# Sahar-E/NeRF-and-DietNeRF

Measured on AMD Instinct MI355X. Metric: rays/sec (coarse+fine) at 256x256, 64 coarse + 128 fine samples, higher is better.
Workload: dtype f16 (3-pass hi/lo split operands, f32 accumulate; fp32-class results)

## Files before the change

### nerf_and_dietnerf_amd/csrc/mlp_f16_frag.h

```cpp
#pragma once
#include "mlp_common.h"

namespace nerf {

typedef _Float16 h8 __attribute__((ext_vector_type(8)));
typedef _Float16 h2 __attribute__((ext_vector_type(2)));
typedef uint32_t frag4 __attribute__((ext_vector_type(4)));

template <int OFF>
__device__ __forceinline__ void lds_read_frag_asm(f32x4& dst, uint32_t base) {
    asm volatile("ds_read_b128 %0, %1 offset:%2" : "=a"(dst) : "v"(base), "n"(OFF) : "memory");
}
template <int N>
__device__ __forceinline__ void lds_wait_frag_asm(f32x4& reg) {
#ifdef NERF_DIAG_NO_LDSWAIT
    asm volatile("" : "+a"(reg) : : "memory");
#else
    asm volatile("s_waitcnt lgkmcnt(%1)" : "+a"(reg) : "n"(N) : "memory");
#endif
}

__device__ __forceinline__ uint32_t pack_h2(float a, float b) {
    const h2 t = {(_Float16)a, (_Float16)b};
    return __builtin_bit_cast(uint32_t, t);
}

constexpr int kHCQ = 32;
constexpr int kHRing = 4;
constexpr int kHChunkBytes = kHCQ * kQuadBytes;
static_assert(kHRing * kHChunkBytes == kRingBytes, "fp16 ring must fill the shared LDS carve");

__device__ __forceinline__ void split_trunc(float y, float& hi_f, float& lo_f) {
    hi_f = __uint_as_float(__float_as_uint(y) & 0xFFFFE000u);
    lo_f = y - hi_f;
}


#ifndef NERF_PE_LX
#define NERF_PE_LX 5
#endif
constexpr int kPeLx = NERF_PE_LX;
constexpr int kPeDim = 3 + 6 * kPeLx;
constexpr int kHStepsPE = (kPeDim + 15) / 16;
constexpr int kHStepsHid = 16;
constexpr int kHStepsDir = 2;
constexpr int kHQpuPE = 2 * kHStepsPE;
constexpr int kHQpuHid = 2 * kHStepsHid;
constexpr int kHQpuSkip = kHQpuPE + kHQpuHid;
constexpr int kHQpuLast = kHQpuHid + 2 * kHStepsDir;
constexpr int kHTilesLast = 5;
constexpr int kHChunksPE = (8 * kHQpuPE + kHCQ - 1) / kHCQ;
constexpr int kHChunksHid = (8 * kHQpuHid) / kHCQ;
constexpr int kHChunksSkip = (8 * kHQpuSkip + kHCQ - 1) / kHCQ;
constexpr int kHChunksLast = (kHTilesLast * kHQpuLast + kHCQ - 1) / kHCQ;
constexpr int kHStreamChunks = kHChunksPE + 6 * kHChunksHid + kHChunksSkip + kHChunksLast;
constexpr int kHChunksSig = (kHQpuLast + kHCQ - 1) / kHCQ;
constexpr int kHStreamChunksSig = kHStreamChunks - kHChunksLast + kHChunksSig;
static_assert(kHStreamChunksSig * (size_t)kHChunkBytes == kStreamBytesF16Sig, "sigma-only stream size mismatch");
constexpr int kFChunksPE = (8 * kHStepsPE + kHCQ - 1) / kHCQ;
constexpr int kFChunksHid = (8 * kHStepsHid) / kHCQ;
constexpr int kFChunksSkip = (8 * (kHStepsPE + kHStepsHid) + kHCQ - 1) / kHCQ;
constexpr int kFChunksLast = (kHTilesLast * (kHStepsHid + kHStepsDir) + kHCQ - 1) / kHCQ;
constexpr int kFStreamChunks = kFChunksPE + 6 * kFChunksHid + kFChunksSkip + kFChunksLast;
static_assert(kFStreamChunks * (size_t)kHChunkBytes == kStreamBytesF16Hi, "hi-only stream size mismatch");
constexpr int kHConstBias = 0;
constexpr int kHConstBias8 = 2048;
constexpr int kHConstBiasSig = 2176;
constexpr int kHConstWrgb = 2208;
constexpr int kHConstBHead = 2592;
constexpr int kHConstFloats = 2608;

static_assert(kHStreamChunks * (size_t)kHChunkBytes == kStreamBytesF16, "stream size mismatch");
constexpr int kXChunksHidSig = (9 * kHQpuHid) / kHCQ;
constexpr int kXChunksLast0 = (4 * kHQpuHid) / kHCQ;
constexpr int kXStreamChunks = kHChunksPE + 6 * kHChunksHid + kHChunksSkip + kXChunksHidSig + kXChunksLast0;
constexpr int kXFChunksHidSig = (9 * kHStepsHid + kHCQ - 1) / kHCQ;
constexpr int kXFChunksLast0 = (4 * kHStepsHid) / kHCQ;
constexpr int kXFStreamChunks = kFChunksPE + 6 * kFChunksHid + kFChunksSkip + kXFChunksHidSig + kXFChunksLast0;
static_assert(kXStreamChunks * (size_t)kHChunkBytes == kStreamBytesF16Xyz, "xyz-only stream size mismatch");
static_assert(kXFStreamChunks * (size_t)kHChunkBytes == kStreamBytesF16HiXyz, "xyz-only hi stream size mismatch");
constexpr int kXConstBiasSig = 2048;
constexpr int kXConstBias8 = 2080;
constexpr int kXConstBias9 = 2336;
constexpr int kXConstWrgb = 2464;
constexpr int kXConstBHead = 2848;
constexpr int kXConstWsig = 2864;
constexpr int kXConstFloats = 3120;
static_assert(kXConstFloats <= kConstFloats, "xyz-only constants must fit the shared LDS carve");
enum { BODY_HIDSIG = 4, BODY_LAST0 = 5, BODY_SIG = 6 };
static_assert(kHConstFloats <= kConstFloats, "f16x3 constants must fit the shared LDS carve");

template <class T>
__device__ __forceinline__ void stream_store(T* p, const T& v) {
#ifndef NERF_STASH_NO_NT
    __builtin_nontemporal_store(v, p);
#else
    *p = v;
#endif
}
__device__ __forceinline__ void stream_store(uint2* p, const uint2& v) {
    typedef uint32_t u32x2 __attribute__((ext_vector_type(2)));
    u32x2 w;
    w[0] = v.x; w[1] = v.y;
    stream_store(reinterpret_cast<u32x2*>(p), w);
}

__device__ __forceinline__ uint32_t mask_push(uint32_t word, uint32_t packed_pair) {
    return (packed_pair & 0x80008000u) | (word >> 1);
}
__host__ __device__ constexpr int mask_bit(int ut, int r) { return 8 * (ut & 1) + (r >> 1) + 16 * (r & 1); }

__host__ __device__ inline int frag_feature(int n, int e, int h) {
    const int t = n >> 1, s = n & 1;
    return 32 * t + 16 * s + 8 * (e >> 2) + 4 * h + (e & 3);
}

}
```

### nerf_and_dietnerf_amd/csrc/mlp_f16x3.hip

```cpp
#include "mlp_f16_frag.h"

#include <math.h>
#include <string.h>

#if defined(NERF_BF16) && NERF_PE_LX == 5
namespace nerf::bf16 {
#elif defined(NERF_BF16)
namespace nerf::bf16::wide {
#elif NERF_PE_LX == 5
namespace nerf {
#else
namespace nerf::wide {
#endif

#ifdef NERF_BF16
typedef __bf16 e8 __attribute__((ext_vector_type(8)));
typedef __bf16 bf2 __attribute__((ext_vector_type(2)));
#define NERF_MFMA_E16 __builtin_amdgcn_mfma_f32_32x32x16_bf16
__device__ __forceinline__ void split_e(float y, float& hi_f, float& lo_f) {
    hi_f = __uint_as_float(__float_as_uint(y) & 0xFFFF0000u);
    lo_f = y - hi_f;
}
__device__ __forceinline__ uint32_t pack_hi(float a, float b) {
    return __builtin_amdgcn_perm(__float_as_uint(b), __float_as_uint(a), 0x07060302u);
}
__device__ __forceinline__ uint32_t pack_lo(float a, float b) {
    const bf2 t = {(__bf16)a, (__bf16)b};
    return __builtin_bit_cast(uint32_t, t);
}
#else
typedef h8 e8;
#define NERF_MFMA_E16 __builtin_amdgcn_mfma_f32_32x32x16_f16
__device__ __forceinline__ void split_e(float y, float& hi_f, float& lo_f) { split_trunc(y, hi_f, lo_f); }
__device__ __forceinline__ uint32_t pack_hi(float a, float b) { return pack_h2(a, b); }
__device__ __forceinline__ uint32_t pack_lo(float a, float b) { return pack_h2(a, b); }
#endif

#ifdef NERF_STAMPS
__device__ unsigned long long g_stamps_h[16];
#endif

template <int BODY, bool PENDING, bool FAST, bool STASH = false, int ROT = 0>
__device__ __forceinline__ void layer_body_h(Pipe& p, uint32_t lane16, uint32_t cb_h, int bias_off_bytes,
                                             float alpha, float* st_prev, float* st_cur, frag4* mk_prev_ptr,
                                             frag4* mk_cur_ptr, frag4& mk_prev, frag4& mk_cur, f32x16 (&accs)[4],
                                             frag4 (&xh)[16], frag4 (&xl)[16], frag4 (&nh)[14], frag4 (&nl)[14],
                                             const frag4 (&peh)[kHStepsPE], const frag4 (&pel)[kHStepsPE], const frag4 (&dh)[2],
                                             const frag4 (&dl)[2], float (&xc)[64], float& sigma_raw) {
    constexpr int NU = BODY == BODY_LAST ? kHTilesLast : BODY == BODY_SIG ? 1 : BODY == BODY_HIDSIG ? 9 : BODY == BODY_LAST0 ? 4 : 8;
    constexpr int NSTEP = BODY == BODY_PE ? kHStepsPE : (BODY == BODY_HID || BODY == BODY_HIDSIG || BODY == BODY_LAST0) ? kHStepsHid
                          : BODY == BODY_SKIP ? kHStepsPE + kHStepsHid : kHStepsHid + kHStepsDir;
    constexpr int SIG0 = BODY == BODY_HIDSIG ? 1 : 0;
    constexpr int TPS = FAST ? 1 : 2;
    constexpr int QPU = TPS * NSTEP;
    constexpr int NQ = NU * QPU;
#ifndef NERF_KPF
#define NERF_KPF 4
#endif
#ifndef NERF_KPF_FAST
#define NERF_KPF_FAST 8
#endif
    constexpr int kPf = FAST ? NERF_KPF_FAST : NERF_KPF;
#ifndef NERF_STASH_EXTRA_FAST
#define NERF_STASH_EXTRA_FAST 0
#endif
#ifndef NERF_STASH_EXTRA_3P
#define NERF_STASH_EXTRA_3P 0
#endif
    constexpr int kStashExtra = STASH ? (FAST ? NERF_STASH_EXTRA_FAST : NERF_STASH_EXTRA_3P) : 0;
    f32x4 pf[kPf];
    const int ck0 = p.ck;
    uint32_t rdbase[2];
    rdbase[0] = lane16 + (uint32_t)((ck0 + 0) & (kHRing - 1)) * kHChunkBytes;
    rdbase[1] = lane16 + (uint32_t)((ck0 + 1) & (kHRing - 1)) * kHChunkBytes;
    auto issue_read = [&](auto qc) {
        constexpr int Qa = decltype(qc)::value;
        lds_read_frag_asm<(Qa % kHCQ) * kQuadBytes>(pf[Qa % kPf], rdbase[(Qa / kHCQ) & 1]);
    };
    static_for<0, kPf>([&](auto ic) {
        if constexpr (decltype(ic)::value < NQ) issue_read(ic);
    });

    auto act = [&](float v) -> float {
        const float av = alpha * v;
        float y;
        asm("v_max_f32 %0, %1, %2" : "=v"(y) : "v"(v), "v"(av));
        return y;
    };
    auto load_bias = [&](int off_bytes, f32x16& dst) {
        static_for<0, 4>([&](auto gc) {
            constexpr int g = decltype(gc)::value;
            const f32x4 b = lds_read4(cb_h + off_bytes + g * 32);
            dst[4 * g + 0] = b[0]; dst[4 * g + 1] = b[1]; dst[4 * g + 2] = b[2]; dst[4 * g + 3] = b[3];
        });
    };
    float sq0 = 0.f, sq1 = 0.f;
    (void)sq0; (void)sq1;
    auto stash4 = [&](auto utc, auto rc, float y0, float y1, float* base) {
        constexpr int ut = decltype(utc)::value;
        constexpr int r = decltype(rc)::value;
        if constexpr ((r & 3) == 0) { sq0 = y0; sq1 = y1; }
        else {
            f32x4 v;
            v[0] = sq0; v[1] = sq1; v[2] = y0; v[3] = y1;
#ifndef NERF_DIAG_NO_STASH_STORES
            stream_store(reinterpret_cast<f32x4*>(base + 32 * (32 * ut + 8 * (r >> 2))), v);
#else
            asm volatile("" :: "v"(v), "v"(base));
#endif
        }
    };
    uint32_t sqh = 0u;
    (void)sqh;
    auto stash4h = [&](auto utc, auto rc, uint32_t ph, float* base) {
        constexpr int ut = decltype(utc)::value;
        constexpr int r = decltype(rc)::value;
        if constexpr ((r & 3) == 0) sqh = ph;
#ifndef NERF_DIAG_NO_STASH_STORES
        else stream_store(reinterpret_cast<uint2*>(reinterpret_cast<uint16_t*>(base) + 32 * (32 * ut + 8 * (r >> 2))), make_uint2(sqh, ph));
#else
        else asm volatile("" :: "v"(sqh), "v"(ph), "v"(base));
#endif
    };
    auto store_pair = [&](auto utc, auto rc, float y0, float y1, auto dest_sel, auto pend_sel) {
        constexpr int ut = decltype(utc)::value;
        constexpr int r = decltype(rc)::value;
        constexpr int n = 2 * ut + (r >> 3), e = r & 7;
        uint32_t ph, pl = 0u;
        if constexpr (FAST) {
            ph = pack_h2(y0, y1);
        } else {
            float h0, l0, h1, l1;
            split_e(y0, h0, l0);
            split_e(y1, h1, l1);
            ph = pack_hi(h0, h1); pl = pack_lo(l0, l1);
        }
        if constexpr (STASH) {
            if constexpr (FAST) stash4h(utc, rc, ph, decltype(pend_sel)::value ? st_prev : st_cur);
            else stash4(utc, rc, y0, y1, decltype(pend_sel)::value ? st_prev : st_cur);
            if constexpr (decltype(pend_sel)::value) mk_prev[ut >> 1] = mask_push(mk_prev[ut >> 1], ph);
            else mk_cur[ut >> 1] = mask_push(mk_cur[ut >> 1], ph);
        }
        if constexpr (decltype(dest_sel)::value) { xh[n][e >> 1] = ph; if constexpr (!FAST) xl[n][e >> 1] = pl; }
        else { nh[n][e >> 1] = ph; if constexpr (!FAST) nl[n][e >> 1] = pl; }
    };

#ifndef NERF_FAST_PACKED_EPI
#define NERF_FAST_PACKED_EPI 1
#endif
    constexpr bool kPackedEpi = FAST && NERF_FAST_PACKED_EPI != 0;
    const uint32_t alpha2 = pack_h2(alpha, alpha);
    (void)alpha2;
    auto act_pair = [&](float v0, float v1) -> uint32_t {
        const uint32_t pk = pack_h2(v0, v1);
        uint32_t q, y;
        asm("v_pk_mul_f16 %0, %1, %2" : "=v"(q) : "v"(pk), "v"(alpha2));
        asm("v_pk_max_f16 %0, %1, %2" : "=v"(y) : "v"(pk), "v"(q));
        return y;
    };
    auto store_pair_p = [&](auto utc, auto rc, uint32_t ph, auto dest_sel, auto pend_sel) {
        constexpr int ut = decltype(utc)::value;
        constexpr int r = decltype(rc)::value;
        constexpr int n = 2 * ut + (r >> 3), e = r & 7;
        if constexpr (STASH) {
            stash4h(utc, rc, ph, decltype(pend_sel)::value ? st_prev : st_cur);
            if constexpr (decltype(pend_sel)::value) mk_prev[ut >> 1] = mask_push(mk_prev[ut >> 1], ph);
            else mk_cur[ut >> 1] = mask_push(mk_cur[ut >> 1], ph);
        }
        if constexpr (decltype(dest_sel)::value) xh[n][e >> 1] = ph;
        else nh[n][e >> 1] = ph;
    };
    (void)act_pair; (void)store_pair_p;
    float ycarry = 0.f;
    (void)ycarry;
    static_for<0, NU>([&](auto uc) {
        constexpr int u = decltype(uc)::value;
        f32x16& acc = accs[(u + ROT) & 3];
        f32x16& prv = accs[(u + ROT + 3) & 3];
        f32x16& nxt = accs[(u + ROT + 1) & 3];
        if constexpr (u == 0 && !PENDING) load_bias(bias_off_bytes, acc);
        static_for<0, NSTEP>([&](auto nc) {
            constexpr int n = decltype(nc)::value;
            f32x4 araw[2];
            static_for<0, TPS>([&](auto tc) {
                constexpr int t = decltype(tc)::value;
                constexpr int Q = u * QPU + TPS * n + t;
                constexpr int left = NQ - Q;
                (void)left;
                constexpr int qc = Q % kHCQ;
                if constexpr (qc == 0 && Q > 0) p.ck += 1;
                if constexpr (qc == kHCQ / 2) {
                    constexpr int room = (NQ - 1 - Q) / 2;
                    pipe_sync_c<kHCQ, kHRing, (room + 1 < kHCQ / 4 ? room + 1 : kHCQ / 4), kStashExtra>(p);
                }
                if constexpr (qc > kHCQ / 2 && (qc - kHCQ / 2) % 2 == 0) {
                    constexpr int Qs = Q - (qc - kHCQ / 2);
                    constexpr bool tail = (NQ - 1 - Qs) / 2 + 1 < kHCQ / 4;
                    pipe_piece_c<(qc - kHCQ / 2) / 2, tail>(p);
                }
                lds_wait_frag_asm<(NQ - Q >= kPf ? kPf - 1 : NQ - Q - 1)>(pf[Q % kPf]);
                araw[t] = pf[Q % kPf];
                if constexpr (Q + kPf < NQ) {
                    constexpr int Qn = Q + kPf;
                    if constexpr (Qn % kHCQ == 0)
                        rdbase[(Qn / kHCQ) & 1] = lane16 + (uint32_t)((ck0 + Qn / kHCQ) & (kHRing - 1)) * kHChunkBytes;
                    issue_read(std::integral_constant<int, Qn>{});
                }
            });
            const e8 a_hi = __builtin_bit_cast(e8, araw[0]);
            const e8 a_lo = __builtin_bit_cast(e8, araw[FAST ? 0 : 1]);
            (void)a_lo;
            frag4 bh_, bl_;
            if constexpr (BODY == BODY_PE) { bh_ = peh[n]; bl_ = pel[n]; }
            else if constexpr (BODY == BODY_HID || BODY == BODY_HIDSIG || BODY == BODY_LAST0) { bh_ = xh[n]; bl_ = xl[n]; }
            else if constexpr (BODY == BODY_SKIP) {
                if constexpr (n < kHStepsPE) { bh_ = peh[n]; bl_ = pel[n]; }
                else { bh_ = xh[n - kHStepsPE]; bl_ = xl[n - kHStepsPE]; }
            } else {
                if constexpr (n < kHStepsHid) { bh_ = xh[n]; bl_ = xl[n]; }
                else { bh_ = dh[n - kHStepsHid]; bl_ = dl[n - kHStepsHid]; }
            }
            const e8 b_hi = __builtin_bit_cast(e8, bh_), b_lo = __builtin_bit_cast(e8, bl_);
            constexpr bool kPend = (u == 0) && PENDING && n < 8;
            constexpr bool kPrevS = (u > SIG0) && BODY != BODY_PE && NSTEP >= 16 && n < 16;
            constexpr int et = kPend ? 7 : (u > SIG0 ? u - 1 - SIG0 : 0);
            constexpr bool kXc = (BODY == BODY_LAST || BODY == BODY_LAST0) && kPrevS;
            if constexpr (BODY == BODY_HIDSIG && u == 1 && n == 0) sigma_raw = prv[0];
            if constexpr (!FAST) {
                acc = NERF_MFMA_E16(a_hi, b_lo, acc, 0, 0, 0);
                acc = NERF_MFMA_E16(a_lo, b_hi, acc, 0, 0, 0);
            }
            acc = NERF_MFMA_E16(a_hi, b_hi, acc, 0, 0, 0);
            if constexpr (kPend && kPackedEpi) {
                constexpr int er = 2 * n;
                store_pair_p(std::integral_constant<int, 7>{}, std::integral_constant<int, er>{}, act_pair(prv[er], prv[er + 1]), std::true_type{}, std::true_type{});
            } else if constexpr (kPrevS && !kXc && kPackedEpi) {
                if constexpr ((n & 1) == 1)
                    store_pair_p(std::integral_constant<int, et>{}, std::integral_constant<int, n - 1>{}, act_pair(prv[n - 1], prv[n]), std::false_type{}, std::false_type{});
            } else if constexpr (kPend) {
                constexpr int er = 2 * n;
                const float y0 = act(prv[er]), y1 = act(prv[er + 1]);
                store_pair(std::integral_constant<int, 7>{}, std::integral_constant<int, er>{}, y0, y1, std::true_type{}, std::true_type{});
            } else if constexpr (kPrevS) {
                const float y = act(prv[n]);
                if constexpr (kXc) {
                    xc[et * 16 + n] = y;
                    if constexpr (STASH) {
                        if constexpr ((n & 1) == 0) ycarry = y;
                        else {
                            const uint32_t pp = pack_h2(ycarry, y);
                            if constexpr (FAST) stash4h(std::integral_constant<int, et>{}, std::integral_constant<int, n - 1>{}, pp, st_cur);
                            else stash4(std::integral_constant<int, et>{}, std::integral_constant<int, n - 1>{}, ycarry, y, st_cur);
                            mk_cur[et >> 1] = mask_push(mk_cur[et >> 1], pp);
                        }
                    }
                }
                else if constexpr ((n & 1) == 0) ycarry = y;
                else store_pair(std::integral_constant<int, et>{}, std::integral_constant<int, n - 1>{}, ycarry, y, std::false_type{}, std::false_type{});
            }
            if constexpr (u == 0 && PENDING) {
                if constexpr (STASH && n == 8) { if (mk_prev_ptr) stream_store(mk_prev_ptr, mk_prev); }
                if constexpr (n == 8) { xh[12] = nh[12]; xl[12] = nl[12]; }
                if constexpr (n == 9) { xh[13] = nh[13]; xl[13] = nl[13]; }
            }
            if constexpr (n == (NSTEP >= 12 ? 10 : 0)) {
                if constexpr (u + 1 < NU) load_bias(bias_off_bytes + (u + 1) * 128, nxt);
                else if constexpr (BODY != BODY_LAST && BODY != BODY_LAST0 && BODY != BODY_SIG) load_bias(bias_off_bytes + NU * 128, nxt);
            }
            if constexpr (BODY == BODY_PE && u > 0 && n == 0) {
                static_for<0, 8>([&](auto pc) {
                    constexpr int r = 2 * decltype(pc)::value;
                    if constexpr (kPackedEpi) {
                        const uint32_t ph = act_pair(prv[r], prv[r + 1]);
                        if constexpr (u - 1 <= 5) store_pair_p(std::integral_constant<int, u - 1>{}, std::integral_constant<int, r>{}, ph, std::true_type{}, std::false_type{});
                        else store_pair_p(std::integral_constant<int, u - 1>{}, std::integral_constant<int, r>{}, ph, std::false_type{}, std::false_type{});
                        return;
                    }
                    const float z0 = act(prv[r]), z1 = act(prv[r + 1]);
                    if constexpr (u - 1 <= 5) store_pair(std::integral_constant<int, u - 1>{}, std::integral_constant<int, r>{}, z0, z1, std::true_type{}, std::false_type{});
                    else store_pair(std::integral_constant<int, u - 1>{}, std::integral_constant<int, r>{}, z0, z1, std::false_type{}, std::false_type{});
                });
            }
            if constexpr ((BODY == BODY_HID || BODY == BODY_SKIP || BODY == BODY_HIDSIG) && u == NU - 1) {
                constexpr int m = BODY == BODY_SKIP ? n - kHStepsPE : n;
                if constexpr (m >= 1 && m - 1 < 12) { xh[m - 1] = nh[m - 1]; xl[m - 1] = nl[m - 1]; }
            }
        });
    });
    if constexpr (BODY == BODY_LAST0) {
        f32x16& lastacc = accs[(NU - 1 + ROT) & 3];
#pragma unroll
        for (int r = 0; r < 16; ++r) xc[(NU - 1) * 16 + r] = act(lastacc[r]);
        if constexpr (STASH) {
            static_for<0, 8>([&](auto pc) {
                constexpr int r = 2 * decltype(pc)::value;
                const float y0 = xc[(NU - 1) * 16 + r], y1 = xc[(NU - 1) * 16 + r + 1];
                const uint32_t pp = pack_h2(y0, y1);
                if constexpr (FAST) stash4h(std::integral_constant<int, NU - 1>{}, std::integral_constant<int, r>{}, pp, st_cur);
                else stash4(std::integral_constant<int, NU - 1>{}, std::integral_constant<int, r>{}, y0, y1, st_cur);
                mk_cur[(NU - 1) >> 1] = mask_push(mk_cur[(NU - 1) >> 1], pp);
            });
            if (mk_cur_ptr) stream_store(mk_cur_ptr, mk_cur);
        }
    }
    if constexpr (BODY == BODY_LAST || BODY == BODY_SIG) {
        static_assert(((NU - 1 + ROT) & 3) == 0, "the sigma tile's accumulator");
        sigma_raw = accs[(NU - 1) & 3][0];
        if constexpr (STASH) { if (mk_cur_ptr) stream_store(mk_cur_ptr, mk_cur); }
    }
    if constexpr (NQ % kHCQ != 0 && NQ % kHCQ <= kHCQ / 2) pipe_sync_c<kHCQ, kHRing, 1, kStashExtra>(p);
    p.ck += 1;
}

template <bool FAST>
__device__ __forceinline__ void split8(const float (&v)[8], frag4& hi, frag4& lo) {
#pragma unroll
    for (int e = 0; e < 8; e += 2) {
        if constexpr (FAST) {
            hi[e >> 1] = pack_h2(v[e], v[e + 1]);
            lo[e >> 1] = 0u;
            continue;
        }
        float h0, l0, h1, l1;
        split_e(v[e], h0, l0);
        split_e(v[e + 1], h1, l1);
        hi[e >> 1] = pack_hi(h0, h1);
        lo[e >> 1] = pack_lo(l0, l1);
    }
}

template <bool FAST, bool STASH = false, bool XYZ = false, bool SIGONLY = false>
__device__ __forceinline__ void mlp_f16_body(const MlpArgs& a) {
    static_assert(!SIGONLY || (!FAST && !STASH && !XYZ), "the sigma-only variant is a render kernel of the 3-pass network");
    extern __shared__ __attribute__((aligned(16))) char smem[];
    const int tid = threadIdx.x;
    const int lane = tid & 63;
    const int wave = __builtin_amdgcn_readfirstlane(tid >> 6);
    const int j = lane & 31;
    const int h = lane >> 5;
    const uint32_t lane16 = kLdsRing + lane * 16;
    uint32_t cb_h = kLdsConst + h * 16;
    asm volatile("" : "+v"(cb_h));

    const long long ntiles = (a.M + 127) / 128;
    if ((long long)blockIdx.x >= ntiles) return;

    for (int i = tid; i < (XYZ ? kXConstFloats : kHConstFloats) / 4; i += 256) {
        const bool sig = SIGONLY && i >= kHConstBias8 / 4 && i < (kHConstBias8 + 32) / 4;
        reinterpret_cast<f32x4*>(smem + kLdsConst)[i] =
            reinterpret_cast<const f32x4*>(a.wconst)[sig ? i + (kHConstBiasSig - kHConstBias8) / 4 : i];
    }

    Pipe p;
    p.ck = 0;
    p.src_next = 0;
    p.n_chunks = XYZ ? (FAST ? kXFStreamChunks : kXStreamChunks) : SIGONLY ? kHStreamChunksSig : (FAST ? kFStreamChunks : kHStreamChunks);
    p.wbase = reinterpret_cast<const char*>(a.wstream);
    p.voff = wave * (kHCQ / 4 * kQuadBytes) + lane * 16;
    p.wave_lds = wave * (kHCQ / 4 * kQuadBytes);
    __syncthreads();
#pragma unroll
    for (int c = 0; c < kHRing - 1; ++c) {
        p.cur_src = p.wbase + (size_t)p.src_next * kHChunkBytes;
        p.cur_dst = kLdsRing + c * kHChunkBytes + p.wave_lds;
        p.src_next += 1;
#pragma unroll
        for (int j = 0; j < kHCQ / 4; ++j) dma_piece(p.cur_src, p.voff + j * kQuadBytes, p.cur_dst + j * kQuadBytes);
    }
    asm volatile("s_waitcnt vmcnt(%0)" ::"n"((kHCQ / 4) * (kHRing - 2)) : "memory");
    __builtin_amdgcn_s_barrier();
    asm volatile("" ::: "memory");

    frag4 xh[16], xl[16], nh[14], nl[14], peh[kHStepsPE], pel[kHStepsPE], dh[2], dl[2];
    f32x16 accs[4];
    float xc[64];
    float sigma_raw = 0.f;

    unsigned long long t0 = 0, t1 = 0, acc_t[8] = {0, 0, 0, 0, 0, 0, 0, 0};
    (void)t0; (void)t1; (void)acc_t;
    for (long long tile = blockIdx.x; tile < ntiles; tile += gridDim.x) {
        STAMP(t0);
        const long long m = tile * 128 + wave * 32 + j;
        const bool valid = m < a.M;
        const long long mm = valid ? m : a.M - 1;
        float px, py, pz, dx, dy, dz;
        if (a.mode == 0) {
            const long long ray = mm / a.S;
            const f32x4 o = *reinterpret_cast<const f32x4*>(a.in_a + ray * 4);
            const f32x4 d = *reinterpret_cast<const f32x4*>(a.in_b + ray * 4);
            const float zz = a.z[mm];
            px = __fadd_rn(o[0], __fmul_rn(d[0], zz));
            py = __fadd_rn(o[1], __fmul_rn(d[1], zz));
            pz = __fadd_rn(o[2], __fmul_rn(d[2], zz));
            dx = d[0]; dy = d[1]; dz = d[2];
        } else {
            px = a.in_a[mm * 3 + 0]; py = a.in_a[mm * 3 + 1]; pz = a.in_a[mm * 3 + 2];
            if constexpr (XYZ) { dx = dy = dz = 0.f; }
            else { dx = a.in_b[mm * 3 + 0]; dy = a.in_b[mm * 3 + 1]; dz = a.in_b[mm * 3 + 2]; }
        }
        const float kPi = 3.1415927410125732f;
        float pv[8 * kHStepsPE];
#pragma unroll
        for (int c = 0; c < 3; ++c) {
            const float v = c == 0 ? px : c == 1 ? py : pz;
            if constexpr (FAST) {
                sin_ladder_fp16_modes<kPeLx>(v * kPi, h, &pv[c * kPeLx]);
            } else {
#pragma unroll
                for (int k = 0; k < kPeLx; ++k) pv[c * kPeLx + k] = sin_shifted(v * (kPi * (float)(1 << k)), h);
            }
        }
        if constexpr (kPeLx == 5) {
            pv[15] = h ? 0.f : px; pv[16] = h ? 0.f : py; pv[17] = h ? 0.f : pz;
#pragma unroll
            for (int i = 18; i < 24; ++i) pv[i] = 0.f;
        } else {
            static_assert(kPeLx == 10, "the wide-PE layout holds exactly 10 octaves");
            pv[30] = h ? pz : px; pv[31] = h ? 0.f : py;
        }
#pragma unroll
        for (int n = 0; n < kHStepsPE; ++n) {
            float t8[8];
#pragma unroll
            for (int e = 0; e < 8; ++e) t8[e] = pv[n * 8 + e];
            split8<FAST>(t8, peh[n], pel[n]);
        }
        float dv[16];
#pragma unroll
        for (int c = 0; c < 3; ++c) {
            const float v = c == 0 ? dx : c == 1 ? dy : dz;
            if constexpr (FAST) {
                sin_ladder_fp16_modes<kLd>(v * kPi, h, &dv[c * kLd]);
            } else {
#pragma unroll
                for (int k = 0; k < kLd; ++k) dv[c * kLd + k] = sin_shifted(v * (kPi * (float)(1 << k)), h);
            }
        }
#pragma unroll
        for (int i = 12; i < 16; ++i) dv[i] = 0.f;
#pragma unroll
        for (int n = 0; n < 2; ++n) {
            float t8[8];
#pragma unroll
            for (int e = 0; e < 8; ++e) t8[e] = dv[n * 8 + e];
            split8<FAST>(t8, dh[n], dl[n]);
        }

        auto st_of = [&](int l) -> float* {
            if constexpr (!STASH) return nullptr;
            else {
                const long long row0 = a.diag_wrap ? (long long)(blockIdx.x & 63) * 128 + wave * 32 : tile * 128 + wave * 32;
                const long long off = row0 * (long long)a.st_ld[l] + (h * 32 + j) * 4;
                if constexpr (FAST) return reinterpret_cast<float*>(reinterpret_cast<uint16_t*>(a.st_ptr[l]) + off);
                else return a.st_ptr[l] + off;
            }
        };
        auto mk_of = [&](int l) -> frag4* {
            if constexpr (!STASH) return nullptr;
            else return a.mask_ptr[l] ? reinterpret_cast<frag4*>(a.mask_ptr[l]) + (tile * 128 + wave * 32 + j) * 2 + h
                                      : nullptr;
        };
        frag4 mk_prev = {0u, 0u, 0u, 0u}, mk_cur = {0u, 0u, 0u, 0u};
        frag4 *mk_prev_ptr = nullptr, *mk_cur_ptr = mk_of(0);
        float* st_prev = nullptr;
        float* st_cur = st_of(0);
        STAMP(t1); acc_t[0] += t1 - t0;
        layer_body_h<BODY_PE, false, FAST, STASH>(p, lane16, cb_h, (kHConstBias + 0 * 256) * 4, a.alpha, st_prev, st_cur, mk_prev_ptr, mk_cur_ptr, mk_prev, mk_cur, accs, xh, xl, nh, nl, peh, pel, dh, dl, xc, sigma_raw);
        STAMP(t0); acc_t[1] += t0 - t1;
#pragma unroll 1
        for (int l = 1; l <= 7; ++l) {
            st_prev = st_cur;
            st_cur = st_of(l);
            mk_prev_ptr = mk_cur_ptr; mk_cur_ptr = mk_of(l);
            mk_prev = mk_cur; mk_cur = frag4{0u, 0u, 0u, 0u};
            if (l == 4) {
                layer_body_h<BODY_SKIP, true, FAST, STASH>(p, lane16, cb_h, (kHConstBias + 4 * 256) * 4, a.alpha, st_prev, st_cur, mk_prev_ptr, mk_cur_ptr, mk_prev, mk_cur, accs, xh, xl, nh, nl, peh, pel, dh, dl, xc, sigma_raw);
                STAMP(t1); acc_t[3] += t1 - t0; t0 = t1;
            } else {
                layer_body_h<BODY_HID, true, FAST, STASH>(p, lane16, cb_h, (kHConstBias + l * 256) * 4, a.alpha, st_prev, st_cur, mk_prev_ptr, mk_cur_ptr, mk_prev, mk_cur, accs, xh, xl, nh, nl, peh, pel, dh, dl, xc, sigma_raw);
                STAMP(t1); acc_t[2] += t1 - t0; t0 = t1;
            }
        }
        if constexpr (XYZ) {
            st_prev = st_cur; st_cur = st_of(8);
            mk_prev_ptr = mk_cur_ptr; mk_cur_ptr = mk_of(8);
            mk_prev = mk_cur; mk_cur = frag4{0u, 0u, 0u, 0u};
            layer_body_h<BODY_HIDSIG, true, FAST, STASH, 0>(p, lane16, cb_h, kXConstBiasSig * 4, a.alpha, st_prev, st_cur, mk_prev_ptr, mk_cur_ptr, mk_prev, mk_cur, accs, xh, xl, nh, nl, peh, pel, dh, dl, xc, sigma_raw);
            st_prev = st_cur; st_cur = st_of(9);
            mk_prev_ptr = mk_cur_ptr; mk_cur_ptr = mk_of(9);
            mk_prev = mk_cur; mk_cur = frag4{0u, 0u, 0u, 0u};
            layer_body_h<BODY_LAST0, true, FAST, STASH, 1>(p, lane16, cb_h, kXConstBias9 * 4, a.alpha, st_prev, st_cur, mk_prev_ptr, mk_cur_ptr, mk_prev, mk_cur, accs, xh, xl, nh, nl, peh, pel, dh, dl, xc, sigma_raw);
        } else if constexpr (SIGONLY) {
            layer_body_h<BODY_SIG, true, FAST, STASH>(p, lane16, cb_h, kHConstBias8 * 4, a.alpha, st_prev, st_cur, mk_prev_ptr, mk_cur_ptr, mk_prev, mk_cur, accs, xh, xl, nh, nl, peh, pel, dh, dl, xc, sigma_raw);
            STAMP(t1); acc_t[4] += t1 - t0;
        } else {
            st_prev = st_cur;
            st_cur = st_of(8);
            mk_prev_ptr = mk_cur_ptr; mk_cur_ptr = mk_of(8);
            mk_prev = mk_cur; mk_cur = frag4{0u, 0u, 0u, 0u};
            layer_body_h<BODY_LAST, true, FAST, STASH>(p, lane16, cb_h, kHConstBias8 * 4, a.alpha, st_prev, st_cur, mk_prev_ptr, mk_cur_ptr, mk_prev, mk_cur, accs, xh, xl, nh, nl, peh, pel, dh, dl, xc, sigma_raw);
            STAMP(t1); acc_t[4] += t1 - t0;
        }
        if constexpr (SIGONLY) {
            if (valid && h == 0) {
                a.raw[m] = sigma_raw;
                if (a.nonfinite && !(fabsf(sigma_raw) <= 3.0e38f)) atomicAdd(a.nonfinite, 1ull);
            }
            STAMP(t0); acc_t[5] += t0 - t1; acc_t[6] += 1;
            continue;
        }
        float o0 = 0.f, o1 = 0.f, o2 = 0.f;
#pragma unroll
        for (int t = 0; t < 4; ++t) {
#pragma unroll
            for (int g = 0; g < 4; ++g) {
                constexpr int kW = XYZ ? kXConstWrgb : kHConstWrgb;
                const f32x4 w0 = lds_read4(cb_h + (kW + 0 * 128 + t * 32 + g * 8) * 4);
                const f32x4 w1 = lds_read4(cb_h + (kW + 1 * 128 + t * 32 + g * 8) * 4);
                const f32x4 w2 = lds_read4(cb_h + (kW + 2 * 128 + t * 32 + g * 8) * 4);
#pragma unroll
                for (int e = 0; e < 4; ++e) {
                    const float x = xc[t * 16 + g * 4 + e];
                    o0 = fmaf(w0[e], x, o0);
                    o1 = fmaf(w1[e], x, o1);
                    o2 = fmaf(w2[e], x, o2);
                }
            }
        }
        o0 += __shfl_xor(o0, 32);
        o1 += __shfl_xor(o1, 32);
        o2 += __shfl_xor(o2, 32);
        const f32x4 bh = lds_read4(kLdsConst + (XYZ ? kXConstBHead : kHConstBHead) * 4);
        if (valid && h == 0) {
            f32x4 out;
            out[0] = o0 + bh[0]; out[1] = o1 + bh[1]; out[2] = o2 + bh[2]; out[3] = sigma_raw;
            *reinterpret_cast<f32x4*>(a.raw + m * 4) = out;
            const float chk = out[0] + out[1] + out[2] + out[3];
            if (a.nonfinite && !(fabsf(chk) <= 3.0e38f)) atomicAdd(a.nonfinite, 1ull);
        }
        STAMP(t0); acc_t[5] += t0 - t1; acc_t[6] += 1;
    }
#ifdef NERF_STAMPS
    if (blockIdx.x == 0 && tid == 0)
        for (int i = 0; i < 8; ++i) g_stamps_h[i] = acc_t[i];
#endif
    asm volatile("s_waitcnt vmcnt(0)" ::: "memory");
}

#ifdef NERF_BF16
__global__ __launch_bounds__(256, 1) void mlp_bf16x3_kernel(const MlpArgs a) { mlp_f16_body<false>(a); }
__global__ __launch_bounds__(256, 1) void mlp_bf16x3_xyz_kernel(const MlpArgs a) { mlp_f16_body<false, false, true>(a); }
#if NERF_PE_LX == 5
__global__ __launch_bounds__(256, 1) void mlp_bf16x3_sig_kernel(const MlpArgs a) { mlp_f16_body<false, false, false, true>(a); }
#endif

static int bf_grid(const MlpArgs& a, int num_cus) {
    const long long ntiles = (a.M + 127) / 128;
    return (int)(ntiles < (long long)num_cus ? ntiles : (long long)num_cus);
}
void launch_mlp_bf16x3(const MlpArgs& a, int num_cus, hipStream_t stream, bool xyz_only) {
    if (a.M <= 0) return;
    if (xyz_only) hipLaunchKernelGGL(mlp_bf16x3_xyz_kernel, dim3(bf_grid(a, num_cus)), dim3(256), kLdsTotal, stream, a);
    else hipLaunchKernelGGL(mlp_bf16x3_kernel, dim3(bf_grid(a, num_cus)), dim3(256), kLdsTotal, stream, a);
}
#if NERF_PE_LX == 5
void launch_mlp_bf16x3_sig(const MlpArgs& a, int num_cus, hipStream_t stream) {
    if (a.M <= 0) return;
    hipLaunchKernelGGL(mlp_bf16x3_sig_kernel, dim3(bf_grid(a, num_cus)), dim3(256), kLdsTotal, stream, a);
}
#endif
void mlp_bf16x3_set_attributes() {
    (void)hipFuncSetAttribute(reinterpret_cast<const void*>(mlp_bf16x3_kernel),
                              hipFuncAttributeMaxDynamicSharedMemorySize, kLdsTotal);
    (void)hipFuncSetAttribute(reinterpret_cast<const void*>(mlp_bf16x3_xyz_kernel),
                              hipFuncAttributeMaxDynamicSharedMemorySize, kLdsTotal);
#if NERF_PE_LX == 5
    (void)hipFuncSetAttribute(reinterpret_cast<const void*>(mlp_bf16x3_sig_kernel),
                              hipFuncAttributeMaxDynamicSharedMemorySize, kLdsTotal);
#endif
}
#else
__global__ __launch_bounds__(256, 1) void mlp_f16x3_kernel(const MlpArgs a) { mlp_f16_body<false>(a); }
__global__ __launch_bounds__(256, 1) void mlp_f16_kernel(const MlpArgs a) { mlp_f16_body<true>(a); }
// ... 141 lines not shown
    return (c == 0 ? 0 : 1) * 8 + 2 * k + h;
}
struct HLayer { const float* k; const float* b; int in, out; };
}

template <class EmitW, class EmitC>
static void pack_f16_map(int n_angles, bool hi_only, EmitW emit_w, EmitC emit_c, bool sig_only = false) {
    const int kd = 256 + 8 * (n_angles + 1);
    const bool xyz_only = n_angles == 0;
    const int shapes_dir[12][2] = {{kPeDim, 256}, {256, 256}, {256, 256}, {256, 256}, {kPeDim + 256, 256}, {256, 256},
                                   {256, 256}, {256, 256}, {kd, 128}, {128, 3}, {kd, 1}, {0, 0}};
    const int shapes_xyz[12][2] = {{kPeDim, 256}, {256, 256}, {256, 256}, {256, 256}, {kPeDim + 256, 256}, {256, 256},
                                   {256, 256}, {256, 256}, {256, 256}, {256, 128}, {128, 3}, {256, 1}};
    const int (*shapes)[2] = xyz_only ? shapes_xyz : shapes_dir;
    struct Lay { long long k, b; int in, out; } L[12];
    long long off = 0;
    for (int i = 0; i < (xyz_only ? 12 : 11); ++i) {
        L[i].in = shapes[i][0]; L[i].out = shapes[i][1];
        L[i].k = off; off += (long long)L[i].in * L[i].out;
        L[i].b = off; off += L[i].out;
    }
    size_t chunk = 0;
    auto emit_body = [&](int layer, int body) {
        const int NU = body == BODY_LAST ? kHTilesLast : body == BODY_SIG ? 1 : body == BODY_HIDSIG ? 9 : body == BODY_LAST0 ? 4 : 8;
        const int NSTEP = body == BODY_PE ? kHStepsPE : (body == BODY_HID || body == BODY_HIDSIG || body == BODY_LAST0) ? kHStepsHid
                          : body == BODY_SKIP ? kHStepsPE + kHStepsHid : kHStepsHid + kHStepsDir;
        const long long b0 = (long long)chunk * (kHChunkBytes / 2);
        for (int u = 0; u < NU; ++u)
            for (int n = 0; n < NSTEP; ++n)
                for (int lane = 0; lane < 64; ++lane)
                    for (int e = 0; e < 8; ++e) {
                        const int i = lane & 31, h = lane >> 5;
                        int row;
                        if (body == BODY_PE) row = h_pe_row(n * 8 + e, h);
                        else if (body == BODY_HID || body == BODY_HIDSIG || body == BODY_LAST0) row = h_hid_row(n, e, h);
                        else if (body == BODY_SKIP) {
                            if (n < kHStepsPE) row = h_pe_row(n * 8 + e, h);
                            else row = kPeDim + h_hid_row(n - kHStepsPE, e, h);
                        } else {
                            if (n < kHStepsHid) row = h_hid_row(n, e, h);
                            else { const int r = h_dir_row((n - kHStepsHid) * 8 + e, h, n_angles); row = r < 0 ? -1 : kHidden + r; }
                        }
                        long long src = -1;
                        if (row >= 0) {
                            if ((body == BODY_LAST && u == kHTilesLast - 1) || body == BODY_SIG)
                                src = i == 0 ? L[10].k + row : -1;
                            else if (body == BODY_HIDSIG && u == 0) src = i == 0 ? L[11].k + row : -1;
                            else if (body == BODY_HIDSIG) src = L[layer].k + (long long)row * L[layer].out + 32 * (u - 1) + i;
                            else src = L[layer].k + (long long)row * L[layer].out + 32 * u + i;
                        }
                        if (hi_only) {
                            emit_w(b0 + (long long)(u * NSTEP + n) * (kQuadBytes / 2) + lane * 8 + e, -1LL, src);
                        } else {
                            const long long q = (long long)(u * NSTEP + n) * 2;
                            emit_w(b0 + (q + 0) * (kQuadBytes / 2) + lane * 8 + e, b0 + (q + 1) * (kQuadBytes / 2) + lane * 8 + e, src);
                        }
                    }
        chunk += (NU * NSTEP * (hi_only ? 1 : 2) + kHCQ - 1) / kHCQ;
    };
    emit_body(0, BODY_PE);
    for (int l = 1; l <= 3; ++l) emit_body(l, BODY_HID);
    emit_body(4, BODY_SKIP);
    for (int l = 5; l <= 7; ++l) emit_body(l, BODY_HID);
    for (int l = 0; l < 8; ++l)
        for (int f = 0; f < 256; ++f) emit_c(kHConstBias + l * 256 + f, L[l].b + f);
    if (xyz_only) {
        emit_body(8, BODY_HIDSIG);
        emit_body(9, BODY_LAST0);
        emit_c(kXConstBiasSig + 0, L[11].b);
        for (int f = 0; f < 256; ++f) emit_c(kXConstBias8 + f, L[8].b + f);
        for (int f = 0; f < 128; ++f) emit_c(kXConstBias9 + f, L[9].b + f);
        for (int c = 0; c < 3; ++c)
            for (int f = 0; f < 128; ++f) emit_c(kXConstWrgb + c * 128 + f, L[10].k + f * 3 + c);
        for (int c = 0; c < 3; ++c) emit_c(kXConstBHead + c, L[10].b + c);
        for (int f = 0; f < 256; ++f) emit_c(kXConstWsig + f, L[11].k + f);
        return;
    }
    emit_body(8, sig_only ? BODY_SIG : BODY_LAST);
    for (int f = 0; f < 128; ++f) emit_c(kHConstBias8 + f, L[8].b + f);
    emit_c(kHConstBiasSig + 0, L[10].b);
    for (int c = 0; c < 3; ++c)
        for (int f = 0; f < 128; ++f) emit_c(kHConstWrgb + c * 128 + f, L[9].k + f * 3 + c);
    for (int c = 0; c < 3; ++c) emit_c(kHConstBHead + c, L[9].b + c);
}

static void pack_weights_f16_impl(const float* blob, int n_angles, void* stream_out, float* const_out, bool hi_only,
                                  bool sig_only = false) {
    memset(stream_out, 0, sig_only ? kStreamBytesF16Sig : n_angles == 0 ? (hi_only ? kStreamBytesF16HiXyz : kStreamBytesF16Xyz)
                                                                        : (hi_only ? kStreamBytesF16Hi : kStreamBytesF16));
    memset(const_out, 0, kConstBytes);
    uint16_t* base = reinterpret_cast<uint16_t*>(stream_out);
    pack_f16_map(n_angles, hi_only,
                 [&](long long ph, long long pl, long long src) {
                     const float w = src < 0 ? 0.f : blob[src];
                     const uint16_t hi = f32_to_e16(w);
                     base[ph] = hi;
                     if (pl >= 0) base[pl] = f32_to_e16(w - e16_to_f32(hi));
                 },
                 [&](long long pos, long long src) { const_out[pos] = blob[src]; }, sig_only);
}

#if defined(NERF_BF16) && NERF_PE_LX == 5
__global__ void repack_bf16x3_kernel(const float* __restrict__ blob, const int32_t* __restrict__ stream_idx,
                                     uint16_t* __restrict__ stream, size_t n_slots) {
    const size_t i = (size_t)blockIdx.x * blockDim.x + threadIdx.x;
    if (i >= n_slots) return;
    const int32_t t = stream_idx[i];
    uint16_t out = 0;
    if (t != 0) {
        const float w = blob[(t >> 1) - 1];
        const __bf16 hi = (__bf16)w;
        const __bf16 v = (t & 1) ? (__bf16)(w - (float)hi) : hi;
        out = __builtin_bit_cast(uint16_t, v);
    }
    stream[i] = out;
}
void launch_repack_bf16x3(const float* blob, const int32_t* stream_idx, void* stream, size_t stream_bytes, hipStream_t s) {
    const size_t n = stream_bytes / 2;
    hipLaunchKernelGGL(repack_bf16x3_kernel, dim3((unsigned)((n + 255) / 256)), dim3(256), 0, s, blob, stream_idx,
                       reinterpret_cast<uint16_t*>(stream), n);
}
void pack_weights_bf16x3_sig(const float* blob, int n_angles, void* stream_out, float* const_out) {
    pack_weights_f16_impl(blob, n_angles, stream_out, const_out, false, true);
}
#endif
#ifdef NERF_BF16
void pack_weights_bf16x3(const float* blob, int n_angles, void* stream_out, float* const_out) {
    pack_weights_f16_impl(blob, n_angles, stream_out, const_out, false);
}
#else
size_t f16_stream_bytes(int n_angles, bool hi_only) {
    if (n_angles == 0) return hi_only ? kStreamBytesF16HiXyz : kStreamBytesF16Xyz;
    return hi_only ? kStreamBytesF16Hi : kStreamBytesF16;
}

void build_f16x3_gather(int n_angles, bool hi_only, int32_t* stream_idx ,
                        int32_t* const_idx ) {
    memset(stream_idx, 0, (f16_stream_bytes(n_angles, hi_only) / 2) * sizeof(int32_t));
    memset(const_idx, 0, kConstFloats * sizeof(int32_t));
    pack_f16_map(n_angles, hi_only,
                 [&](long long ph, long long pl, long long src) {
                     if (src < 0) return;
                     stream_idx[ph] = (int32_t)(2 * (src + 1));
                     if (pl >= 0) stream_idx[pl] = (int32_t)(2 * (src + 1) + 1);
                 },
                 [&](long long pos, long long src) { const_idx[pos] = (int32_t)(src + 1); });
}

__global__ void repack_f16x3_kernel(const float* __restrict__ blob, const int32_t* __restrict__ stream_idx,
                                    uint16_t* __restrict__ stream, const int32_t* __restrict__ const_idx,
                                    float* __restrict__ cst, size_t n_slots) {
    const size_t i = (size_t)blockIdx.x * blockDim.x + threadIdx.x;
    if (i < n_slots) {
        const int32_t t = stream_idx[i];
        uint16_t out = 0;
        if (t != 0) {
            const float w = blob[(t >> 1) - 1];
            const _Float16 hi = (_Float16)w;
            const _Float16 v = (t & 1) ? (_Float16)(w - (float)hi) : hi;
            out = __builtin_bit_cast(uint16_t, v);
        }
        stream[i] = out;
    }
    if (i < (size_t)kConstFloats) {
        const int32_t t = const_idx[i];
        cst[i] = t ? blob[t - 1] : 0.f;
// ... 35 lines not shown
```

Baseline: 1.759 million.

## Compute sigma head with per-lane FMA dot product instead of extra MFMA tile

In the 3-pass fp16 render path, the sigma output no longer runs through a dedicated MFMA tile streamed from the weight ring. Each lane instead accumulates a dot product of its hi/lo activation fragments with sigma weights held in the LDS constant area, reduced with one cross-lane shuffle. This drops one tile's worth of LDS fragment reads and MFMAs per layer. In exchange it adds scalar FMAs and extra constant loads, and for BODY_SIG it first has to activate and store layer 7's outputs up front.

```diff
diff --git a/nerf_and_dietnerf_amd/csrc/mlp_f16_frag.h b/nerf_and_dietnerf_amd/csrc/mlp_f16_frag.h
--- a/nerf_and_dietnerf_amd/csrc/mlp_f16_frag.h
+++ b/nerf_and_dietnerf_amd/csrc/mlp_f16_frag.h
@@ -69,6 +69,9 @@
 constexpr int kHConstWrgb = 2208;
 constexpr int kHConstBHead = 2592;
 constexpr int kHConstFloats = 2608;
+constexpr int kHConstWsig = 2608;
+constexpr int kHConstFloatsCin = 2896;
+static_assert(kHConstFloatsCin <= kConstFloats, "f16x3 constants must fit the shared LDS carve");
 
 static_assert(kHStreamChunks * (size_t)kHChunkBytes == kStreamBytesF16, "stream size mismatch");
 constexpr int kXChunksHidSig = (9 * kHQpuHid) / kHCQ;
diff --git a/nerf_and_dietnerf_amd/csrc/mlp_f16x3.hip b/nerf_and_dietnerf_amd/csrc/mlp_f16x3.hip
--- a/nerf_and_dietnerf_amd/csrc/mlp_f16x3.hip
+++ b/nerf_and_dietnerf_amd/csrc/mlp_f16x3.hip
@@ -40,7 +40,7 @@
 __device__ unsigned long long g_stamps_h[16];
 #endif
 
-template <int BODY, bool PENDING, bool FAST, bool STASH = false, int ROT = 0>
+template <int BODY, bool PENDING, bool FAST, bool STASH = false, int ROT = 0, bool CIN = false>
 __device__ __forceinline__ void layer_body_h(Pipe& p, uint32_t lane16, uint32_t cb_h, int bias_off_bytes,
                                              float alpha, float* st_prev, float* st_cur, frag4* mk_prev_ptr,
                                              frag4* mk_cur_ptr, frag4& mk_prev, frag4& mk_cur, f32x16 (&accs)[4],
@@ -54,6 +54,9 @@
     constexpr int TPS = FAST ? 1 : 2;
     constexpr int QPU = TPS * NSTEP;
     constexpr int NQ = NU * QPU;
+    constexpr bool kSigV = CIN && (BODY == BODY_LAST || BODY == BODY_SIG);
+    constexpr int NUC = kSigV ? NU - 1 : NU;
+    constexpr int NQC = NUC * QPU;
 #ifndef NERF_KPF
 #define NERF_KPF 4
 #endif
@@ -78,7 +81,7 @@
         lds_read_frag_asm<(Qa % kHCQ) * kQuadBytes>(pf[Qa % kPf], rdbase[(Qa / kHCQ) & 1]);
     };
     static_for<0, kPf>([&](auto ic) {
-        if constexpr (decltype(ic)::value < NQ) issue_read(ic);
+        if constexpr (decltype(ic)::value < NQC) issue_read(ic);
     });
 
     auto act = [&](float v) -> float {
@@ -173,6 +176,39 @@
     (void)act_pair; (void)store_pair_p;
     float ycarry = 0.f;
     (void)ycarry;
+    float sg[4] = {0.f, 0.f, 0.f, 0.f};
+    (void)sg;
+    auto sig_step = [&](auto gc) {
+        constexpr int g = decltype(gc)::value;
+        constexpr int f = g >> 2, d = g & 3;
+        uint32_t ph, pl;
+        if constexpr (f < kHStepsHid) { ph = xh[f][d]; pl = xl[f][d]; }
+        else { ph = dh[f - kHStepsHid][d]; pl = dl[f - kHStepsHid][d]; }
+        const h2 vh = __builtin_bit_cast(h2, ph), vl = __builtin_bit_cast(h2, pl);
+        extern __shared__ __attribute__((aligned(16))) char smem[];
+        typedef float f32x2 __attribute__((ext_vector_type(2)));
+        const f32x2 w = *reinterpret_cast<const f32x2*>(smem + cb_h + (kHConstWsig + f * 16 + (d >> 1) * 8 + 2 * (d & 1)) * 4);
+        const float w0 = w[0], w1 = w[1];
+        float s = sg[d];
+        s = __builtin_fmaf((float)vh[0], w0, s);
+        s = __builtin_fmaf((float)vl[0], w0, s);
+        s = __builtin_fmaf((float)vh[1], w1, s);
+        s = __builtin_fmaf((float)vl[1], w1, s);
+        sg[d] = s;
+    };
+    (void)sig_step;
+    if constexpr (kSigV && BODY == BODY_SIG) {
+        static_assert(PENDING && !STASH, "BODY_SIG follows layer 7 of a render kernel");
+        f32x16& prv7 = accs[(ROT + 3) & 3];
+        static_for<0, 8>([&](auto pc) {
+            constexpr int er = 2 * decltype(pc)::value;
+            const float y0 = act(prv7[er]), y1 = act(prv7[er + 1]);
+            store_pair(std::integral_constant<int, 7>{}, std::integral_constant<int, er>{}, y0, y1, std::true_type{}, std::true_type{});
+        });
+        xh[12] = nh[12]; xl[12] = nl[12];
+        xh[13] = nh[13]; xl[13] = nl[13];
+        static_for<0, 4 * (kHStepsHid + kHStepsDir)>(sig_step);
+    }
     static_for<0, NU>([&](auto uc) {
         constexpr int u = decltype(uc)::value;
         f32x16& acc = accs[(u + ROT) & 3];
@@ -198,15 +234,17 @@
                     constexpr bool tail = (NQ - 1 - Qs) / 2 + 1 < kHCQ / 4;
                     pipe_piece_c<(qc - kHCQ / 2) / 2, tail>(p);
                 }
-                lds_wait_frag_asm<(NQ - Q >= kPf ? kPf - 1 : NQ - Q - 1)>(pf[Q % kPf]);
+                if constexpr (Q >= NQC) return;
+                lds_wait_frag_asm<(NQC - Q >= kPf ? kPf - 1 : NQC - Q - 1)>(pf[Q % kPf]);
                 araw[t] = pf[Q % kPf];
-                if constexpr (Q + kPf < NQ) {
+                if constexpr (Q + kPf < NQC) {
                     constexpr int Qn = Q + kPf;
                     if constexpr (Qn % kHCQ == 0)
                         rdbase[(Qn / kHCQ) & 1] = lane16 + (uint32_t)((ck0 + Qn / kHCQ) & (kHRing - 1)) * kHChunkBytes;
                     issue_read(std::integral_constant<int, Qn>{});
                 }
             });
+            if constexpr (u >= NUC) return;
             const e8 a_hi = __builtin_bit_cast(e8, araw[0]);
             const e8 a_lo = __builtin_bit_cast(e8, araw[FAST ? 0 : 1]);
             (void)a_lo;
@@ -264,7 +302,7 @@
                 if constexpr (n == 9) { xh[13] = nh[13]; xl[13] = nl[13]; }
             }
             if constexpr (n == (NSTEP >= 12 ? 10 : 0)) {
-                if constexpr (u + 1 < NU) load_bias(bias_off_bytes + (u + 1) * 128, nxt);
+                if constexpr (u + 1 < NUC) load_bias(bias_off_bytes + (u + 1) * 128, nxt);
                 else if constexpr (BODY != BODY_LAST && BODY != BODY_LAST0 && BODY != BODY_SIG) load_bias(bias_off_bytes + NU * 128, nxt);
             }
             if constexpr (BODY == BODY_PE && u > 0 && n == 0) {
@@ -281,6 +319,7 @@
                     else store_pair(std::integral_constant<int, u - 1>{}, std::integral_constant<int, r>{}, z0, z1, std::false_type{}, std::false_type{});
                 });
             }
+            if constexpr (kSigV && u < NUC) sig_step(std::integral_constant<int, u * NSTEP + n>{});
             if constexpr ((BODY == BODY_HID || BODY == BODY_SKIP || BODY == BODY_HIDSIG) && u == NU - 1) {
                 constexpr int m = BODY == BODY_SKIP ? n - kHStepsPE : n;
                 if constexpr (m >= 1 && m - 1 < 12) { xh[m - 1] = nh[m - 1]; xl[m - 1] = nl[m - 1]; }
@@ -303,7 +342,17 @@
             if (mk_cur_ptr) stream_store(mk_cur_ptr, mk_cur);
         }
     }
-    if constexpr (BODY == BODY_LAST || BODY == BODY_SIG) {
+    if constexpr (kSigV && BODY == BODY_LAST) {
+        static_assert(!STASH, "CIN is a render path");
+        f32x16& lastacc = accs[(NUC - 1 + ROT) & 3];
+#pragma unroll
+        for (int r = 0; r < 16; ++r) xc[(NUC - 1) * 16 + r] = act(lastacc[r]);
+    }
+    if constexpr (kSigV) {
+        float s = (sg[0] + sg[1]) + (sg[2] + sg[3]);
+        s += __shfl_xor(s, 32);
+        sigma_raw = s + lds_read4(kLdsConst + kHConstBiasSig * 4)[0];
+    } else if constexpr (BODY == BODY_LAST || BODY == BODY_SIG) {
         static_assert(((NU - 1 + ROT) & 3) == 0, "the sigma tile's accumulator");
         sigma_raw = accs[(NU - 1) & 3][0];
         if constexpr (STASH) { if (mk_cur_ptr) stream_store(mk_cur_ptr, mk_cur); }
@@ -332,6 +381,11 @@
 template <bool FAST, bool STASH = false, bool XYZ = false, bool SIGONLY = false>
 __device__ __forceinline__ void mlp_f16_body(const MlpArgs& a) {
     static_assert(!SIGONLY || (!FAST && !STASH && !XYZ), "the sigma-only variant is a render kernel of the 3-pass network");
+#if defined(NERF_BF16) || NERF_PE_LX != 5
+    constexpr bool kCin = false;
+#else
+    constexpr bool kCin = !FAST && !STASH && !XYZ;
+#endif
     extern __shared__ __attribute__((aligned(16))) char smem[];
     const int tid = threadIdx.x;
     const int lane = tid & 63;
@@ -345,7 +399,7 @@
     const long long ntiles = (a.M + 127) / 128;
     if ((long long)blockIdx.x >= ntiles) return;
 
-    for (int i = tid; i < (XYZ ? kXConstFloats : kHConstFloats) / 4; i += 256) {
+    for (int i = tid; i < (XYZ ? kXConstFloats : kCin ? kHConstFloatsCin : kHConstFloats) / 4; i += 256) {
         const bool sig = SIGONLY && i >= kHConstBias8 / 4 && i < (kHConstBias8 + 32) / 4;
         reinterpret_cast<f32x4*>(smem + kLdsConst)[i] =
             reinterpret_cast<const f32x4*>(a.wconst)[sig ? i + (kHConstBiasSig - kHConstBias8) / 4 : i];
@@ -491,14 +545,14 @@
             mk_prev = mk_cur; mk_cur = frag4{0u, 0u, 0u, 0u};
             layer_body_h<BODY_LAST0, true, FAST, STASH, 1>(p, lane16, cb_h, kXConstBias9 * 4, a.alpha, st_prev, st_cur, mk_prev_ptr, mk_cur_ptr, mk_prev, mk_cur, accs, xh, xl, nh, nl, peh, pel, dh, dl, xc, sigma_raw);
         } else if constexpr (SIGONLY) {
-            layer_body_h<BODY_SIG, true, FAST, STASH>(p, lane16, cb_h, kHConstBias8 * 4, a.alpha, st_prev, st_cur, mk_prev_ptr, mk_cur_ptr, mk_prev, mk_cur, accs, xh, xl, nh, nl, peh, pel, dh, dl, xc, sigma_raw);
+            layer_body_h<BODY_SIG, true, FAST, STASH, 0, kCin>(p, lane16, cb_h, kHConstBias8 * 4, a.alpha, st_prev, st_cur, mk_prev_ptr, mk_cur_ptr, mk_prev, mk_cur, accs, xh, xl, nh, nl, peh, pel, dh, dl, xc, sigma_raw);
             STAMP(t1); acc_t[4] += t1 - t0;
         } else {
             st_prev = st_cur;
             st_cur = st_of(8);
             mk_prev_ptr = mk_cur_ptr; mk_cur_ptr = mk_of(8);
             mk_prev = mk_cur; mk_cur = frag4{0u, 0u, 0u, 0u};
-            layer_body_h<BODY_LAST, true, FAST, STASH>(p, lane16, cb_h, kHConstBias8 * 4, a.alpha, st_prev, st_cur, mk_prev_ptr, mk_cur_ptr, mk_prev, mk_cur, accs, xh, xl, nh, nl, peh, pel, dh, dl, xc, sigma_raw);
+            layer_body_h<BODY_LAST, true, FAST, STASH, 0, kCin>(p, lane16, cb_h, kHConstBias8 * 4, a.alpha, st_prev, st_cur, mk_prev_ptr, mk_cur_ptr, mk_prev, mk_cur, accs, xh, xl, nh, nl, peh, pel, dh, dl, xc, sigma_raw);
             STAMP(t1); acc_t[4] += t1 - t0;
         }
         if constexpr (SIGONLY) {
@@ -806,6 +860,14 @@
     for (int c = 0; c < 3; ++c)
         for (int f = 0; f < 128; ++f) emit_c(kHConstWrgb + c * 128 + f, L[9].k + f * 3 + c);
     for (int c = 0; c < 3; ++c) emit_c(kHConstBHead + c, L[9].b + c);
+    for (int f = 0; f < kHStepsHid + kHStepsDir; ++f)
+        for (int e = 0; e < 8; ++e)
+            for (int h = 0; h < 2; ++h) {
+                int row;
+                if (f < kHStepsHid) row = h_hid_row(f, e, h);
+                else { const int r = h_dir_row((f - kHStepsHid) * 8 + e, h, n_angles); row = r < 0 ? -1 : kHidden + r; }
+                if (row >= 0) emit_c(kHConstWsig + f * 16 + (e >> 2) * 8 + h * 4 + (e & 3), L[10].k + row);
+            }
 }
 
 static void pack_weights_f16_impl(const float* blob, int n_angles, void* stream_out, float* const_out, bool hi_only,
```

Result: no change. 1.754 million (-0.3%).
